# tomstrident/GAN-based-Video-Style-Transfer

Measured on NVIDIA B200. Metric: warped frame-pairs/sec, higher is better.
Workload: dtype f32

## Files before the change

### gan-based-video-style-transfer_b200/_cabi.py

```python
import ctypes
import os
import subprocess

_HERE = os.path.dirname(os.path.abspath(__file__))
CSRC = os.path.join(_HERE, "csrc")
LIB_PATH = os.environ.get("TCL_B200_LIB") or os.path.join(CSRC, "libtcl_b200.so")
HEADER = os.path.join(os.path.dirname(_HERE), "include", "tcl_b200.h")
ABI_VERSION = 6

F32, BF16 = 0, 1
OCC, MOB, VALIDITY = 1, 2, 4
L2, L1 = 0, 1
FIN_MEAN, FIN_RMSE = 0, 1

NVCC_FLAGS = ["-gencode", "arch=compute_100a,code=sm_100a", "-O3", "-lineinfo", "-std=c++17",
              "-Xcompiler", "-fPIC", "-shared"]
SOURCES = ["tcl_kernels.cu", "tcl_host.cu", "tcl_cv2.cu", "tcl_agg.cu", "tcl_chain.cu"]
HEADERS = ["tcl_math.cuh", "tcl_common.cuh"]


class TclArgs(ctypes.Structure):
    _fields_ = [
        ("ff", ctypes.c_void_p), ("bf", ctypes.c_void_p), ("mask_in", ctypes.c_void_p),
        ("prev", ctypes.c_void_p), ("cur", ctypes.c_void_p),
# ... 81 lines not shown
    "tclb200_warp_backward": (_c.c_int, [_vp, _vp, _vp, _vp, _vp, _i, _i, _i, _i, _i, _vp]),
    "tclb200_fbcheck": (_c.c_int, [_vp, _vp, _vp, _i, _i, _i, _i, _vp, _vp]),
    "tclb200_tcl_forward": (_c.c_int, [_c.POINTER(TclArgs), _vp]),
    "tclb200_host_workspace_bytes": (_c.c_size_t, [_i, _i, _i, _i, _i, _i, _i, _i]),
    "tclb200_tcl_forward_host": (_c.c_int, [_c.POINTER(HostArgs), _vp]),
    "tclb200_tcl_backward": (_c.c_int, [_vp, _vp, _vp, _vp, _vp, _vp, _vp, _i, _i, _i, _i, _i, _i, _vp]),
    "tclb200_tcl_backward_scaled": (_c.c_int, [_vp, _vp, _vp, _vp, _vp, _c.c_float, _vp, _vp, _i, _i, _i, _i, _i, _i, _vp]),
    "tclb200_backward_workspace_bytes": (_c.c_size_t, [_i, _i, _i, _i, _i]),
    "tclb200_warp_backward_dt": (_c.c_int, [_vp, _vp, _vp, _vp, _vp, _i, _i, _i, _i, _i, _i, _vp, _c.c_size_t, _vp]),
    "tclb200_tcl_backward_dt": (_c.c_int, [_vp, _vp, _vp, _vp, _vp, _c.c_float, _vp, _vp, _i, _i, _i, _i, _i, _i, _i, _vp,
                                           _c.c_size_t, _vp]),
    "tclb200_hwc_split": (_c.c_int, [_vp, _i, _i, _i, _i, _i, _vp, _vp, _vp, _vp]),
    "tclb200_occlusion_u8_to_mask": (_c.c_int, [_vp, _vp, _c.c_size_t, _vp]),
    "tclb200_upsample_flow": (_c.c_int, [_vp, _vp, _vp, _i, _i, _i, _vp]),
    "tclb200_cv2_remap": (_c.c_int, [_vp, _vp, _vp, _i, _i, _i, _i, _vp]),
    "tclb200_cv2_fb_check": (_c.c_int, [_vp, _vp, _vp, _i, _i, _i, _i, _i, _vp, _vp]),
    "tclb200_reconet_scratch_bytes": (_c.c_size_t, [_i, _i, _i]),
    "tclb200_reconet_loss": (_c.c_int, [_vp, _vp, _vp, _vp, _vp, _vp, _vp, _vp, _vp, _vp, _c.c_size_t, _i, _i, _i, _vp]),
    "tclb200_ruder_input": (_c.c_int, [_vp, _vp, _vp, _vp, _vp, _vp, _i, _i, _i, _vp]),
    "tclb200_pack_sequence_sums": (_c.c_int, [_vp, _vp, _vp, _i, _i, _c.c_double, _vp, _vp]),
    "tclb200_unpack_sequence_means": (_c.c_int, [_vp, _i, _vp, _vp]),
    "tclb200_debug_force_generic": (None, [_i]),
    "tclb200_debug_tile_stats": (_c.c_int, [_vp, _i]),
    "tclb200_debug_launch_count": (_c.c_ulonglong, [_i]),
}

_lib = None


class TclB200Error(RuntimeError):
    pass


def lib():
    global _lib
    if _lib is not None:
        return _lib
    if not os.path.exists(LIB_PATH):
        raise TclB200Error(
            f"{LIB_PATH} is missing: build it with `python -c 'import __graft_entry__ as g; g.build()'` "
            "(nvcc, sm_100a). There is no CPU or PyTorch fallback for this path.")
    handle = ctypes.CDLL(LIB_PATH)
    for name, (res, args) in _PROTOTYPES.items():
        fn = getattr(handle, name)
        fn.restype, fn.argtypes = res, args
    got = handle.tclb200_abi_version()
# ... 19 lines not shown
```

### gan-based-video-style-transfer_b200/csrc/tcl_kernels.cu

```cuda
#include <cuda.h>
#include <cuda_bf16.h>
#include <cuda_runtime.h>
#include <limits.h>
#include <stdint.h>
#include <stdio.h>
#include <string.h>
#include <type_traits>

#include "../../include/tcl_b200.h"
#include "tcl_common.cuh"
#include "tcl_math.cuh"

#ifndef TCL_TH
#define TCL_TH 32
#endif
#ifndef TCL_BH
#define TCL_BH 42
#endif
#ifndef TCL_BH8
#define TCL_BH8 44
#endif
#ifndef TCL_BH16
#define TCL_BH16 TCL_BH
#endif
#ifndef TCL_BW
#define TCL_BW 80
#endif
#ifndef TCL_BW16
#define TCL_BW16 80
#endif
#ifndef TCL_NS
#define TCL_NS 2
#endif
#ifndef TCL_NB
#define TCL_NB (TCL_NS + 2)
#endif
#ifndef TCL_NS_NOFF
#define TCL_NS_NOFF 3
#endif
#ifndef TCL_BH_NOFF
#define TCL_BH_NOFF 40
#endif
#ifndef TCL_SCANNERS
#define TCL_SCANNERS 2
#endif
#ifndef TCL_PACKED
// ... 244 lines not shown
        const float xc = to_f32(s_c[c][ii[q]]);
        if (LOSS == TCLB200_L2) {
          const float md = __fmul_rn(keep[q], __fsub_rn(xc, w[q][c]));
          e = __fmaf_rn(md, md, e);
        } else {
          e = __fadd_rn(e, __fmul_rn(keep[q], fabsf(__fsub_rn(w[q][c], xc))));
        }
      }
      err = ok[q] ? e : err;
    }
  }
  double s = warp_sum((double)err);
  if ((threadIdx.x & 31) == 0) s_red[threadIdx.x >> 5] = s;
  __syncthreads();
  if (threadIdx.x == 0) {
    s = 0.0;
#pragma unroll
    for (int k = 0; k < kDirectThreads / 32; ++k) s += s_red[k];
    __stcg(&p.scratch.partials[(size_t)pair * p.tiles_per_pair + chunk], s);
  }
}

__device__ unsigned long long g_tile_stats[2];
#ifdef TCL_TRACE
constexpr int kTraceTiles = 64;
__device__ unsigned long long g_trace[160][kTraceTiles][4];
__device__ __forceinline__ unsigned long long gtime() { unsigned long long t; asm volatile("mov.u64 %0, %globaltimer;" : "=l"(t)); return t; }
#define TCL_STAMP(k, slot) do { if ((k) < kTraceTiles && blockIdx.x < 160) g_trace[blockIdx.x][(k)][(slot)] = gtime(); } while (0)
#else
#define TCL_STAMP(k, slot) do { } while (0)
#endif
#ifdef TCL_CWARPS
constexpr int kCWarpsPacked = TCL_CWARPS, kCWarpsOther = TCL_CWARPS;
#else
constexpr int kCWarpsPacked = 8, kCWarpsOther = 16;
#endif

template <typename FrameT, int CT, int TW_, int TH_, int BW_, int BH_, int NB_, int NS_, int CW_, bool FF_ = true>
struct WsCfg {
  static constexpr int TW = TW_, TH = TH_, BW = BW_, BH = BH_, NB = NB_, NS = NS_;
  static constexpr int CW = CW_;
  static constexpr int kProducerWarp = CW;
  static constexpr int kScannerWarp = CW + 1;
  static constexpr int kScanners = TCL_SCANNERS;
  static constexpr int kThreads = 32 * (CW + 1 + kScanners);
  static constexpr int kHaloL = 4;
  static constexpr int kBfW = TW + 16, kBfH = TH + 2;
  static constexpr int kXAlign = 16 / (int)sizeof(FrameT);
  static constexpr int kRowBlocks = CW / 4;
  static constexpr int kRows = TH / kRowBlocks;
  static constexpr int kPPL = kRows / 2;
  static constexpr int kC = CT > 0 ? CT : 1;
  static constexpr unsigned kBfLoad = 2u * kBfH * kBfW * 4u;
  static constexpr unsigned kFfLoad = 2u * BH * BW * 4u;
  static constexpr unsigned kPrevLoad = (unsigned)(CT > 0 ? CT : 0) * BH * BW * (unsigned)sizeof(FrameT);
  static constexpr size_t kBfStage = align_up(kBfLoad, 128);
  static constexpr size_t kFfStage = FF_ ? align_up(kFfLoad, 128) : 0;
  static constexpr size_t kSrcStage = kFfStage + align_up(kPrevLoad, 128);
  static constexpr size_t kBfOff = 0;
  static constexpr size_t kSrcOff = kBfOff + NB * kBfStage;
  static constexpr size_t kCtlOff = kSrcOff + NS * kSrcStage;
  static constexpr size_t kCtlBytes = 1024 + (size_t)NS * CW * 32 * 4;
  static constexpr size_t kSmemBytes = kCtlOff + kCtlBytes + 128;
  static_assert(TW == 64 && CW % 4 == 0 && TH % kRowBlocks == 0 && kRows % 2 == 0, "lane mapping: 16-column blocks, row pairs");
  static_assert(kBfW % 32 == 16, "flow-tile pitch must be 16 (mod 32) words: adjacent rows fall into disjoint bank halves");
  static_assert((BW * (int)sizeof(FrameT)) % 16 == 0 && BW % 4 == 0, "TMA: box rows are multiples of 16 bytes");
#if TCL_DIAG != 3
  static_assert(NB >= NS + 1, "the flow tile of a tile is scanned NS tiles ahead of its use");
  static_assert(kSmemBytes <= 232448, "a CTA has at most 227 KB of shared memory");
#endif
};
__host__ __device__ constexpr int pix_dy(int k) { return 2 * k; }
template <typename Cfg>
__device__ __forceinline__ void lane_origin(int warp, int lane, int& lx0, int& ly0) {
  lx0 = 16 * (warp & 3) + (lane & 15);
  ly0 = Cfg::kRows * (warp >> 2) + (lane >> 4);
}

struct TileId { int pair, tile, x0, y0, pf, cf, bfi, ffi; };

template <int NB, int NS, int CW>
struct WsCtl {
  uint64_t bf_full[NB], scanned[NB], src_full[NS], done[NS];
  TileId tinfo[NB];
  int meta[NS][4];
  int box[NB][4];
  float red[NS][CW * 32];
};

// ... 708 lines not shown
                                                                  t.x0 + lx0, t.y0 + ly0 + pix_dy(k), 0.0f, 0.0f, 0.0f, 0.0f);
          keepbits = (keepbits & ~(1u << k)) | ((kp != 0.0f ? 1u : 0u) << k);
        }
      }
  }
  if (CT == 0) {
    float* mo = p.mask_out + (size_t)t.pair * gplane + (size_t)(t.y0 + ly0) * g.W + (t.x0 + lx0);
#pragma unroll
    for (int k = 0; k < P; ++k)
      if (!EDGE || (xin && 2 * k < rows_in)) __stcs(mo + (ptrdiff_t)pix_dy(k) * g.W, ((keepbits >> k) & 1u) ? 1.0f : 0.0f);
    return 0.0f;
  }
  float err = 0.0f;
#pragma unroll
  for (int k = 0; k < P; ++k) {
    if (MASK == MASK_GIVEN) err = __fadd_rn(err, e[k]);
    else err = ((keepbits >> k) & 1u) ? __fadd_rn(err, e[k]) : err;
  }
  return err;
}

template <typename FrameT, int MASK, bool REDUCE, int CT, int LEAN, typename Cfg>
__global__ void __launch_bounds__(Cfg::kThreads, 1) fused_forward_ws_kernel(const FwdParams p, const __grid_constant__ CUtensorMap tm_bf,
                                                                         const __grid_constant__ CUtensorMap tm_ff,
                                                                         const __grid_constant__ CUtensorMap tm_prev,
                                                                         const __grid_constant__ CUtensorMap tm_cur) {
  constexpr int NB = Cfg::NB, NS = Cfg::NS, P = Cfg::kPPL;
  constexpr int kCWarps = Cfg::CW;
  constexpr int kLoss = LEAN == 2 ? TCLB200_L1 : TCLB200_L2;
  constexpr bool kPacked = TCL_PACKED && (((LEAN == 1 || LEAN == 2) && CT == 3 && (MASK == MASK_COMPUTED || (MASK == MASK_GIVEN && TCL_PACKED_GIVEN))) ||
                                          (TCL_PACKED_MASK && LEAN == 1 && CT == 0 && MASK == MASK_COMPUTED && !REDUCE));
  using Ctl = WsCtl<NB, NS, kCWarps>;
  static_assert(sizeof(Ctl) <= Cfg::kCtlBytes, "control block too large");
  extern __shared__ __align__(128) unsigned char smem_raw[];
  unsigned char* smem = smem_raw + ((128u - (smem_u32(smem_raw) & 127u)) & 127u);
  Ctl* ctl = reinterpret_cast<Ctl*>(smem + Cfg::kCtlOff);
  auto bf_stage = [&](int s) { return reinterpret_cast<float*>(smem + Cfg::kBfOff + (size_t)s * Cfg::kBfStage); };
  auto ff_stage = [&](int s) { return reinterpret_cast<float*>(smem + Cfg::kSrcOff + (size_t)s * Cfg::kSrcStage); };
  auto prev_stage = [&](int s) { return reinterpret_cast<FrameT*>(smem + Cfg::kSrcOff + (size_t)s * Cfg::kSrcStage + Cfg::kFfStage); };

  const int total_tiles = p.B * p.tiles_per_pair;
  const bool want_occ = MASK == MASK_COMPUTED && (LEAN ? LEAN != 3 : (p.flags & TCLB200_OCC) != 0);
  const bool want_frames = CT > 0 && (LEAN || p.prev != nullptr);
  const bool want_scan = want_occ || want_frames;
  const int warp = threadIdx.x >> 5, lane = threadIdx.x & 31;
  const Geo& g = p.geo;
  auto real = [&](int k) { return ctl->tinfo[k % NB].pair >= 0; };

  if (REDUCE) asm volatile("griddepcontrol.launch_dependents;" ::: "memory");
// ... 8 lines not shown
    const bool dynamic = p.scratch.tile_ctr != nullptr;
    int tg_next = (int)blockIdx.x;
    bool exhausted = false;
    auto next_tile = [&]() {
      const int tg = tg_next;
      tg_next = dynamic ? (int)gridDim.x + (int)atomicAdd(p.scratch.tile_ctr, 1u) : tg + (int)gridDim.x;
      return tg;
    };
    auto issue_bf = [&](int k) {
      const int s = k % NB;
      const int tg = exhausted ? total_tiles : next_tile();
      if (tg >= total_tiles) {
        exhausted = true;
        ctl->tinfo[s].pair = -1;
        mbar_arrive(&ctl->bf_full[s]);
        return;
      }
      const TileId t = tile_id(p, tg, Cfg::TW, Cfg::TH);
      ctl->tinfo[s] = t;
      mbar_expect_tx(&ctl->bf_full[s], Cfg::kBfLoad);
      tma_load_4d(bf_stage(s), &tm_bf, &ctl->bf_full[s], t.x0 - Cfg::kHaloL, t.y0 - 1, 0, t.bfi);
      if (LEAN && CT > 0 && p.cur != nullptr) tma_prefetch_l2_4d(&tm_cur, t.x0, t.y0, 0, t.cf);
    };
    struct Placement { int ox, oy, mode, ffi, pf; };
    auto place_src = [&](int k) -> Placement {
      const int sb = k % NB;
      const TileId t = ctl->tinfo[sb];
      int ox = 0, oy = 0, mode = 0;
#if TCL_DIAG == 3
      if (true) { ox = (t.x0 - 8) & ~3; oy = t.y0 - 4; mode = 1; } else
#endif
      if (want_scan) {
        mbar_wait_idle(&ctl->scanned[sb], (k / NB) & 1);
        const float xmin = ord2f(ctl->box[sb][0]), ymin = ord2f(ctl->box[sb][1]), xmax = ord2f(ctl->box[sb][2]), ymax = ord2f(ctl->box[sb][3]);
        const float lim = 30000.0f;
        const bool sane = xmin > -lim && xmax < lim && ymin > -lim && ymax < lim && xmin <= xmax && ymin <= ymax;
        if (sane) {
          const float i2x = __fmul_rn(2.0f, g.inv_dx), i2y = __fmul_rn(2.0f, g.inv_dy);
          auto coord = [](float a, float i2, float sz) {
            const float tt = __fadd_rn(__fsub_rn(__fmul_rn(a, i2), 1.0f), 1.0f);
            return __fmul_rn(__fmaf_rn(tt, sz, -1.0f), 0.5f);
          };
          const int bx0 = __float2int_rd(coord(xmin, i2x, g.Wf)), bx1 = __float2int_rd(coord(xmax, i2x, g.Wf));
          const int by0 = __float2int_rd(coord(ymin, i2y, g.Hf)), by1 = __float2int_rd(coord(ymax, i2y, g.Hf));
          ox = bx0 & ~(Cfg::kXAlign - 1);
          oy = by0;
          const bool fitx = bx1 + 1 - ox < Cfg::BW, fity = by1 + 1 - oy < Cfg::BH;
          mode = (fitx && fity) ? 1 : 2;
          if (mode == 2) {
            if (!fitx) ox = ((bx0 + bx1 + 1 - Cfg::BW) / 2) & ~(Cfg::kXAlign - 1);
            if (!fity) oy = (by0 + by1 + 1 - Cfg::BH) / 2;
          }
        }
        if (mode != 1) atomicAdd(&g_tile_stats[mode == 2 ? 1 : 0], 1ull);
      }
      return Placement{ox, oy, mode, t.ffi, t.pf};
    };
    auto issue_src = [&](int k, const Placement& pl) {
      const int ss = k % NS;
      ctl->meta[ss][0] = pl.ox; ctl->meta[ss][1] = pl.oy; ctl->meta[ss][2] = pl.mode;
#if TCL_DIAG == 1
      if (false) {
#else
      if (pl.mode != 0) {
#endif
        TCL_STAMP(k, 0);
        mbar_expect_tx(&ctl->src_full[ss], (want_occ ? Cfg::kFfLoad : 0u) + (want_frames ? Cfg::kPrevLoad : 0u));
        if (want_occ) tma_load_4d(ff_stage(ss), &tm_ff, &ctl->src_full[ss], pl.ox, pl.oy, 0, pl.ffi);
        if (want_frames) tma_load_4d(prev_stage(ss), &tm_prev, &ctl->src_full[ss], pl.ox, pl.oy, 0, pl.pf);
      } else {
        mbar_arrive(&ctl->src_full[ss]);
      }
    };

    if (lane == 0) {
      prefetch_tmap(&tm_bf);
      if (want_occ) prefetch_tmap(&tm_ff);
      if (want_frames) prefetch_tmap(&tm_prev);
      for (int j = 0; j < NB; ++j) issue_bf(j);
      for (int j = 0; j < NS && real(j); ++j) issue_src(j, place_src(j));
    }
    __syncwarp();
    for (int j = 0; real(j); ++j) {
      mbar_wait_idle(&ctl->done[j % NS], (j / NS) & 1);
      const TileId t = ctl->tinfo[j % NB];
      double ts = 0.0;
      if (REDUCE) {
        const float* r = ctl->red[j % NS] + lane;
#pragma unroll
        for (int w = 0; w < kCWarps; ++w) ts += (double)r[32 * w];
      }
      __syncwarp();
      if (lane == 0) {
        if (real(j + NS)) issue_src(j + NS, place_src(j + NS));
        issue_bf(j + NB);
      }
      __syncwarp();
      if (REDUCE) {
        ts = warp_sum(ts);
        if (lane == 0) __stcg(&p.scratch.partials[(size_t)t.pair * p.tiles_per_pair + t.tile], ts);
      }
    }
    if (dynamic && lane == 0) {
      __threadfence();
      if (atomicAdd(p.scratch.tile_ctr + 1, 1u) == gridDim.x - 1) {
        p.scratch.tile_ctr[0] = 0;
        p.scratch.tile_ctr[1] = 0;
      }
    }
    return;
  }

  if (warp >= Cfg::kScannerWarp) {
    if (!want_scan || TCL_DIAG == 3) return;
    for (int k = warp - Cfg::kScannerWarp;; k += Cfg::kScanners) {
      const int sb = k % NB;
      mbar_wait_idle(&ctl->bf_full[sb], (k / NB) & 1);
      if (ctl->tinfo[sb].pair < 0) return;
      scan_flow_tile<Cfg>(bf_stage(sb), ctl->tinfo[sb], g, p.row_end, ctl->box[sb], lane);
      __syncwarp();
      if (lane == 0) mbar_arrive(&ctl->scanned[sb]);
    }
  }

  unsigned near = 0;
// ... 455 lines not shown
  if (!batch_stride) batch_stride = plane_stride * planes;
  const cuuint64_t dims[4] = {(cuuint64_t)W, (cuuint64_t)H, (cuuint64_t)planes, (cuuint64_t)B};
  const cuuint64_t strides[3] = {(cuuint64_t)W * esize, (cuuint64_t)plane_stride * esize, (cuuint64_t)batch_stride * esize};
  const cuuint32_t box[4] = {(cuuint32_t)bw, (cuuint32_t)bh, (cuuint32_t)bp, 1u};
  const cuuint32_t estr[4] = {1u, 1u, 1u, 1u};
  const CUtensorMapDataType dt = esize == 2 ? CU_TENSOR_MAP_DATA_TYPE_BFLOAT16 : CU_TENSOR_MAP_DATA_TYPE_FLOAT32;
  return fn(m, dt, 4, const_cast<void*>(base), dims, strides, box, estr, CU_TENSOR_MAP_INTERLEAVE_NONE,
            CU_TENSOR_MAP_SWIZZLE_NONE, CU_TENSOR_MAP_L2_PROMOTION_L2_256B, CU_TENSOR_MAP_FLOAT_OOB_FILL_NONE) == CUDA_SUCCESS;
}

static int sm_count() {
  static int cache[64] = {};
  int dev = 0, v = 0;
  if (cudaGetDevice(&dev) != cudaSuccess) return 148;
  if (dev >= 0 && dev < 64 && cache[dev] > 0) return cache[dev];
  if (cudaDeviceGetAttribute(&v, cudaDevAttrMultiProcessorCount, dev) != cudaSuccess || v <= 0) return 148;
  if (dev >= 0 && dev < 64) cache[dev] = v;
  return v;
}

static cudaError_t launch_fold(const FwdParams& p, cudaStream_t s);

template <typename FrameT, int MASK, bool REDUCE, int CT, int LEAN, int CW>
static cudaError_t launch_tma_cw(const FwdParams& p, const CUtensorMap& tb, const CUtensorMap& tf, const CUtensorMap& tp, const CUtensorMap& tc,
                                 cudaStream_t s) {
  constexpr bool has_ff = MASK == MASK_COMPUTED;
  constexpr int NS = has_ff ? (CT == 0 && LEAN == 1 ? TCL_NS_MASK : TCL_NS) : TCL_NS_NOFF, NB = has_ff ? (CT == 0 && LEAN == 1 ? TCL_NS_MASK + 2 : TCL_NB) : TCL_NS_NOFF + 2;
  using Cfg = WsCfg<FrameT, CT, kTW, kTH, box_width<FrameT>(), (has_ff ? box_height(CW, (int)sizeof(FrameT)) : TCL_BH_NOFF), NB, NS, CW, has_ff>;
  auto kern = fused_forward_ws_kernel<FrameT, MASK, REDUCE, CT, LEAN, Cfg>;
  static bool configured[64] = {};
  int dev = 0;
  if (cudaGetDevice(&dev) != cudaSuccess || dev < 0 || dev >= 64) dev = 63;
  if (!configured[dev] || dev == 63) {
    cudaError_t e = cudaFuncSetAttribute(kern, cudaFuncAttributeMaxDynamicSharedMemorySize, (int)Cfg::kSmemBytes);
    if (e != cudaSuccess) return e;
    configured[dev] = true;
  }
  const size_t tiles = (size_t)p.B * p.tiles_per_pair;
  const size_t slots = (size_t)sm_count();
  const unsigned grid = (unsigned)(tiles < slots ? tiles : slots);
  kern<<<grid, Cfg::kThreads, Cfg::kSmemBytes, s>>>(p, tb, tf, tp, tc);
  ++g_launches;
  cudaError_t e = cudaGetLastError();
  if (e != cudaSuccess || !REDUCE) return e;
  return launch_fold(p, s);
}

template <typename FrameT, int MASK, bool REDUCE, int CT, int LEAN>
static cudaError_t launch_tma(const FwdParams& p, const CUtensorMap& tb, const CUtensorMap& tf, const CUtensorMap& tp, const CUtensorMap& tc,
                              cudaStream_t s) {
  constexpr bool packed8 = TCL_PACKED && MASK == MASK_COMPUTED && sizeof(FrameT) == 4 &&
                           (((LEAN == 1 || LEAN == 2) && CT == 3) || (TCL_PACKED_MASK && LEAN == 1 && CT == 0 && !REDUCE));
  if constexpr (packed8 && kCWarpsPacked != kCWarpsOther) {
    if (p.cw_packed) return launch_tma_cw<FrameT, MASK, REDUCE, CT, LEAN, kCWarpsPacked>(p, tb, tf, tp, tc, s);
  }
  if (p.cw_packed && kCWarpsPacked != kCWarpsOther) return cudaErrorInvalidConfiguration;
  return launch_tma_cw<FrameT, MASK, REDUCE, CT, LEAN, kCWarpsOther>(p, tb, tf, tp, tc, s);
}

static cudaError_t launch_fold(const FwdParams& p, cudaStream_t s) {
  ++g_launches;
  cudaLaunchConfig_t cfg;
  memset(&cfg, 0, sizeof(cfg));
  const bool small = p.B <= kFoldSmallPairs && (size_t)p.B * p.tiles_per_pair <= (size_t)kFoldSmallPartials;
  cfg.gridDim = dim3(small ? 1u : (unsigned)p.B); cfg.blockDim = dim3(small ? 1024 : kThreads); cfg.stream = s;
  cudaLaunchAttribute attr[1];
  attr[0].id = cudaLaunchAttributeProgrammaticStreamSerialization;
  attr[0].val.programmaticStreamSerializationAllowed = 1;
  cfg.attrs = attr; cfg.numAttrs = 1;
  return small ? cudaLaunchKernelEx(&cfg, fold_partials_small_kernel, p) : cudaLaunchKernelEx(&cfg, fold_partials_kernel, p);
}

template <typename FrameT>
static cudaError_t launch_direct(const FwdParams& p, cudaStream_t s) {
  auto kern = p.loss == TCLB200_L1 ? fused_forward_direct_kernel<FrameT, TCLB200_L1> : fused_forward_direct_kernel<FrameT, TCLB200_L2>;
  kern<<<(unsigned)((size_t)p.B * p.tiles_per_pair), kDirectThreads, 0, s>>>(p);
  ++g_launches;
  cudaError_t e = cudaGetLastError();
  if (e != cudaSuccess) return e;
  return launch_fold(p, s);
}

template <typename FrameT, int MASK, bool REDUCE>
static cudaError_t launch_generic(const FwdParams& p, cudaStream_t s) {
  const unsigned grid = (unsigned)((size_t)p.B * p.tiles_per_pair);
  if (p.C == 3) fused_forward_generic_kernel<FrameT, MASK, REDUCE, 3><<<grid, kThreads, 0, s>>>(p);
  else fused_forward_generic_kernel<FrameT, MASK, REDUCE, 0><<<grid, kThreads, 0, s>>>(p);
  ++g_launches;
  return cudaGetLastError();
}

template <typename FrameT>
static cudaError_t dispatch(const FwdParams& p, int mask_kind, bool reduce, bool tma, const CUtensorMap& tb, const CUtensorMap& tf,
                            const CUtensorMap& tp, const CUtensorMap& tc, cudaStream_t s) {
#ifdef TCL_HOT_ONLY
  if (sizeof(FrameT) == (TCL_HOT_ONLY == 2 ? 2 : 4) && mask_kind == MASK_COMPUTED && reduce && tma && p.C == 3 && p.prev && p.cur && !p.warp_out && !p.mask_out &&
      !p.blend_out && !p.near_threshold && p.loss == TCLB200_L2)
    return launch_tma<typename std::conditional<TCL_HOT_ONLY == 2, __nv_bfloat16, float>::type, MASK_COMPUTED, true, 3, 1>(p, tb, tf, tp, tc, s);
  if (mask_kind == MASK_COMPUTED && !reduce && !p.prev) return launch_generic<float, MASK_COMPUTED, false>(p, s);
  return cudaErrorNotSupported;
#else
#define TCL_CASE(MK, RD)                                                                       \
  if (mask_kind == MK && reduce == RD) {                                                       \
    if (!tma) return launch_generic<FrameT, MK, RD>(p, s);                                     \
    if (p.C == 3 && lean_out && MK != MASK_NONE) return launch_tma<FrameT, (MK == MASK_NONE ? MASK_GIVEN : MK), RD, 3, 4>(p, tb, tf, tp, tc, s); \
    if (p.C == 3 && lean && RD) return p.loss == TCLB200_L1 ? launch_tma<FrameT, MK, true, 3, 2>(p, tb, tf, tp, tc, s)   \
                                                            : launch_tma<FrameT, MK, true, 3, 1>(p, tb, tf, tp, tc, s);  \
    if (MK == MASK_COMPUTED && !RD && lean_mask) return launch_tma<float, MASK_COMPUTED, false, 0, 1>(p, tb, tf, tp, tc, s); \
    if (MK == MASK_COMPUTED && !RD && lean_mob) return launch_tma<float, MASK_COMPUTED, false, 0, 3>(p, tb, tf, tp, tc, s); \
    if (MK == MASK_NONE && !RD && lean_warp) return launch_tma<FrameT, MASK_NONE, false, 3, 1>(p, tb, tf, tp, tc, s); \
    return p.C == 3 ? launch_tma<FrameT, MK, RD, 3, 0>(p, tb, tf, tp, tc, s) : launch_tma<FrameT, MK, RD, 0, 0>(p, tb, tf, tp, tc, s); \
  }
  const bool lean = reduce && p.prev && p.cur && !p.warp_out && !p.mask_out && !p.blend_out && !p.near_threshold &&
                    !(p.flags & TCLB200_VALIDITY) && mask_kind != MASK_NONE &&
                    (mask_kind != MASK_COMPUTED || (p.flags & (TCLB200_OCC | TCLB200_MOB)) == (TCLB200_OCC | TCLB200_MOB));
  const bool lean_out = p.prev && p.cur && (p.warp_out || p.blend_out || (p.mask_out && mask_kind == MASK_COMPUTED)) &&
                        !(p.mask_out && mask_kind == MASK_GIVEN) && !p.near_threshold && !(p.flags & TCLB200_VALIDITY) &&
                        p.loss == TCLB200_L2 && mask_kind != MASK_NONE &&
                        (mask_kind != MASK_COMPUTED || (p.flags & (TCLB200_OCC | TCLB200_MOB)) == (TCLB200_OCC | TCLB200_MOB));
  const bool lean_mask = !reduce && !p.prev && p.mask_out && !p.near_threshold && mask_kind == MASK_COMPUTED &&
                         (p.flags & (TCLB200_OCC | TCLB200_MOB)) == (TCLB200_OCC | TCLB200_MOB);
  const bool lean_mob = !reduce && !p.prev && p.mask_out && !p.near_threshold && mask_kind == MASK_COMPUTED &&
                        (p.flags & (TCLB200_OCC | TCLB200_MOB)) == TCLB200_MOB;
  const bool lean_warp = !reduce && p.prev && p.C == 3 && !p.cur && p.warp_out && !p.mask_out && !p.blend_out && mask_kind == MASK_NONE;
  TCL_CASE(MASK_COMPUTED, true)
  TCL_CASE(MASK_COMPUTED, false)
  TCL_CASE(MASK_GIVEN, true)
  TCL_CASE(MASK_GIVEN, false)
  TCL_CASE(MASK_NONE, true)
  TCL_CASE(MASK_NONE, false)
#undef TCL_CASE
  return cudaErrorInvalidValue;
#endif
}

extern "C" int tclb200_debug_tile_stats(unsigned long long* out2, int reset) {
  unsigned long long zero[2] = {0, 0};
  if (out2) CUDA_TRY(cudaMemcpyFromSymbol(out2, tcl::g_tile_stats, sizeof(zero)));
  if (reset) CUDA_TRY(cudaMemcpyToSymbol(tcl::g_tile_stats, zero, sizeof(zero)));
  return TCLB200_OK;
}

extern "C" unsigned long long tclb200_debug_launch_count(int reset) {
  const unsigned long long n = g_launches;
  if (reset) g_launches = 0;
  return n;
}

#ifdef TCL_TRACE
extern "C" int tclb200_debug_trace(unsigned long long* out, size_t bytes) {
  if (bytes > sizeof(tcl::g_trace)) bytes = sizeof(tcl::g_trace);
  CUDA_TRY(cudaMemcpyFromSymbol(out, tcl::g_trace, bytes));
  return TCLB200_OK;
}
#endif

static int g_force_generic = 0;
extern "C" void tclb200_debug_force_generic(int on) { g_force_generic = on; }
#ifndef TCL_DIRECT_MAX_PX
#define TCL_DIRECT_MAX_PX (2u << 20)
#endif

// ... 23 lines not shown
    return fail(TCLB200_ERR_INVALID, "ff given but neither TCLB200_OCC nor TCLB200_MOB requested");
  if (!a->prev && !a->mask_out) return fail(TCLB200_ERR_INVALID, "nothing to compute: no frames and no mask_out");

  const int esz = a->dtype == TCLB200_BF16 ? 2 : 4;
  const size_t hw = (size_t)a->H * a->W;
  const size_t bf_plane = a->bf_plane_stride ? a->bf_plane_stride : hw, bf_batch = a->bf_batch_stride ? a->bf_batch_stride : 2 * bf_plane;
  const size_t ff_plane = a->ff_plane_stride ? a->ff_plane_stride : hw, ff_batch = a->ff_batch_stride ? a->ff_batch_stride : 2 * ff_plane;
  if (bf_plane < hw || ff_plane < hw || (a->B > 1 && (bf_batch < hw || ff_batch < hw)))
    return fail(TCLB200_ERR_INVALID, "flow plane / pair strides must be at least H*W");
  const bool strides16 = bf_plane % 4 == 0 && bf_batch % 4 == 0 && ff_plane % 4 == 0 && ff_batch % 4 == 0;
  bool tma = g_force_generic != 1 && (a->W % 4 == 0) && ((a->W * esz) % 16 == 0) && aligned16(a->bf) && aligned16(a->ff) &&
             aligned16(a->prev) && aligned16(a->cur) && (!a->prev || a->C == 3) && a->B <= 65535 * 16 && strides16 &&
             a->H <= 16384 && a->W <= 16384;
  const bool cw_hot = reduce && a->prev && a->cur && a->C == 3 && !a->warp_out && !a->mask_out && !a->blend_out;
  const bool cw_mask = TCL_PACKED_MASK && !reduce && !a->prev && a->mask_out;
  const bool cw_packed = TCL_PACKED && kCWarpsPacked != kCWarpsOther && tma && a->dtype == TCLB200_F32 && mask_kind == MASK_COMPUTED &&
                         (cw_hot || cw_mask) && !a->near_threshold &&
                         !(a->flags & TCLB200_VALIDITY) && (a->flags & (TCLB200_OCC | TCLB200_MOB)) == (TCLB200_OCC | TCLB200_MOB) &&
                         (size_t)a->H * a->W >= (size_t)384 * 384;
  const size_t launch_px = (size_t)a->B * (size_t)((band ? a->row_end - a->row_begin : a->H)) * a->W;
  const bool direct = tma && g_force_generic != 2 && mask_kind == MASK_GIVEN && reduce && a->C == 3 && !a->warp_out && !a->mask_out &&
                      !a->blend_out && !a->near_threshold && !(a->flags & (TCLB200_VALIDITY | TCLB200_THROUGHPUT)) && aligned16(a->mask_in) &&
                      (launch_px <= TCL_DIRECT_MAX_PX || g_force_generic == 3);
  CUtensorMap tb, tf, tp, tc;
  memset(&tb, 0, sizeof(tb)); memset(&tf, 0, sizeof(tf)); memset(&tp, 0, sizeof(tp)); memset(&tc, 0, sizeof(tc));
  if (tma && !direct) {
    const int bw = a->dtype == TCLB200_BF16 ? box_width<__nv_bfloat16>() : box_width<float>();
    const int kBH = mask_kind == MASK_COMPUTED ? box_height(cw_packed ? kCWarpsPacked : kCWarpsOther, esz) : TCL_BH_NOFF;
    tma = make_map(&tb, a->bf, 4, a->W, a->H, 2, a->bf_index ? a->n_bf_fields : a->B, kTW + 16, kTH + 2, 2, bf_plane, bf_batch);
    if (tma && mask_kind == MASK_COMPUTED && (a->flags & TCLB200_OCC))
      tma = make_map(&tf, a->ff, 4, a->W, a->H, 2, a->ff_index ? a->n_ff_fields : a->B, bw, kBH, 2, ff_plane, ff_batch);
    if (tma && a->prev) tma = make_map(&tp, a->prev, esz, a->W, a->H, 3, a->prev_index ? a->n_prev_frames : a->B, bw, kBH, 3);
    if (tma && a->prev && a->cur) tma = make_map(&tc, a->cur, esz, a->W, a->H, 3, a->cur_index ? a->n_cur_frames : a->B, kTW, kTH, 3);
  }

  FwdParams p;
  memset(&p, 0, sizeof(p));
  p.ff = a->ff; p.bf = a->bf; p.mask_in = a->mask_in; p.prev = a->prev; p.cur = a->cur;
  p.ff_plane = ff_plane; p.ff_batch = ff_batch; p.bf_plane = bf_plane; p.bf_batch = bf_batch;
  p.prev_index = a->prev ? a->prev_index : nullptr; p.cur_index = a->cur ? a->cur_index : nullptr;
  p.bf_index = a->bf_index; p.ff_index = a->ff ? a->ff_index : nullptr;
  p.pair_group = a->pair_group > 1 ? a->pair_group : 1;
  p.cw_packed = cw_packed ? 1 : 0;
  p.warp_out = a->warp_out; p.mask_out = a->mask_out; p.blend_out = a->blend_out;
  p.pair_sums = a->pair_sums; p.total_sums = a->total_sums; p.pair_vals = a->pair_vals; p.total_val = a->total_val;
  p.near_threshold = a->near_threshold;
  p.geo = make_geo(a->H, a->W);
  p.B = a->B; p.C = a->prev ? a->C : 0;
  p.row_begin = band ? a->row_begin : 0;
  p.row_end = band ? a->row_end : a->H;
  p.tiles_x = tma ? cdiv(a->W, kTW) : cdiv(a->W, 32);
  p.tiles_per_pair = p.tiles_x * (tma ? cdiv(p.row_end - p.row_begin, kTH) : cdiv(p.row_end - p.row_begin, kWarps));
  if (direct) { p.tiles_x = 0; p.tiles_per_pair = (int)(((size_t)(p.row_end - p.row_begin) * a->W + kDirectChunk - 1) / kDirectChunk); }
  p.flags = a->flags; p.loss = a->loss; p.finalize = a->finalize;
  p.inv_count = a->prev ? 1.0 / ((double)a->C * a->H * a->W) : 0.0;
  if ((size_t)p.B * p.tiles_per_pair >= 0x7fffffffu) return fail(TCLB200_ERR_UNSUPPORTED, "too many tiles for one launch");
  if (reduce) {
    if (!a->scratch || a->scratch_bytes < tclb200_scratch_bytes(a->B, a->H, a->W))
      return fail(TCLB200_ERR_INVALID, "scratch missing or smaller than tclb200_scratch_bytes(B,H,W)");
    char* base = reinterpret_cast<char*>(a->scratch);
    const size_t tpp_max = (size_t)cdiv(a->W, 32) * cdiv(a->H, kWarps);
    p.scratch.partials = reinterpret_cast<double*>(base);
    p.scratch.pair_ticket = reinterpret_cast<unsigned*>(base + align_up((size_t)a->B * tpp_max * sizeof(double), 256));
    p.scratch.batch_ticket = p.scratch.pair_ticket + a->B;
    const size_t tiles = (size_t)p.B * p.tiles_per_pair;
    p.scratch.tile_ctr = (tma && !direct && tiles > 16 * (size_t)sm_count()) ? p.scratch.batch_ticket + 1 : nullptr;
  }
  if (direct) {
    const cudaError_t e = a->dtype == TCLB200_BF16 ? launch_direct<__nv_bfloat16>(p, s) : launch_direct<float>(p, s);
    if (e != cudaSuccess) return fail(TCLB200_ERR_CUDA, "fused forward (direct) launch: %s", cudaGetErrorString(e));
    return TCLB200_OK;
  }
  const cudaError_t e = a->dtype == TCLB200_BF16 ? dispatch<__nv_bfloat16>(p, mask_kind, reduce, tma, tb, tf, tp, tc, s)
                                                 : dispatch<float>(p, mask_kind, reduce, tma, tb, tf, tp, tc, s);
  if (e != cudaSuccess) return fail(TCLB200_ERR_CUDA, "fused forward launch: %s", cudaGetErrorString(e));
  return TCLB200_OK;
}

extern "C" int tclb200_tcl_forward(const tclb200_tcl_args* args, tclb200_stream_t stream) {
  return run_fused(args, reinterpret_cast<cudaStream_t>(stream));
}

extern "C" int tclb200_warp(const void* x, const float* f, void* out, int B, int C, int H, int W, int dtype, int flags,
                            tclb200_stream_t stream) {
  if (!x || !f || !out) return fail(TCLB200_ERR_INVALID, "x, f and out are required");
  tclb200_tcl_args a;
  memset(&a, 0, sizeof(a));
  a.bf = f; a.prev = x; a.warp_out = out;
  a.B = B; a.C = C; a.H = H; a.W = W; a.dtype = dtype; a.flags = flags & TCLB200_VALIDITY;
  return run_fused(&a, reinterpret_cast<cudaStream_t>(stream));
}

extern "C" int tclb200_fbcheck(const float* ff, const float* bf, float* mask_out, int B, int H, int W, int flags,
                               unsigned long long* near_threshold, tclb200_stream_t stream) {
  if (!bf || !mask_out) return fail(TCLB200_ERR_INVALID, "bf and mask_out are required");
  if ((flags & TCLB200_OCC) && !ff) return fail(TCLB200_ERR_INVALID, "ff is required for the occlusion test");
  if (!(flags & (TCLB200_OCC | TCLB200_MOB))) return fail(TCLB200_ERR_INVALID, "flags must request TCLB200_OCC and/or TCLB200_MOB");
// ... 200 lines not shown
```

### include/tcl_b200.h

```cpp
#ifndef TCL_B200_H_
#define TCL_B200_H_

#include <stddef.h>
#include <stdint.h>

#ifdef __cplusplus
extern "C" {
#endif

#define TCLB200_ABI_VERSION 6

#define TCLB200_OK 0
#define TCLB200_ERR_INVALID 1
#define TCLB200_ERR_CUDA 2
#define TCLB200_ERR_UNSUPPORTED 3

#define TCLB200_F32 0
#define TCLB200_BF16 1

#define TCLB200_OCC 1
#define TCLB200_MOB 2
#define TCLB200_VALIDITY 4
#define TCLB200_THROUGHPUT 8

// ... 97 lines not shown
int tclb200_occlusion_u8_to_mask(const uint8_t* src, float* dst, size_t n, tclb200_stream_t stream);

int tclb200_upsample_flow(const float* flow, const float* mask, float* out, int N, int H, int W, tclb200_stream_t stream);

int tclb200_cv2_remap(const float* src, const float* flow, float* out, int N, int H, int W, int C, tclb200_stream_t stream);
int tclb200_cv2_fb_check(const float* ff, const float* bf, float* mask, int N, int H, int W, int flags, int prewarped,
                         unsigned long long* near_threshold, tclb200_stream_t stream);

size_t tclb200_reconet_scratch_bytes(int B, int H, int W);
int tclb200_reconet_loss(const float* flow, const float* mask, const float* styled1, const float* styled2, const float* img1,
                         const float* img2, float* lum_out, float* loss_out, double* sum_out, void* scratch, size_t scratch_bytes,
                         int B, int H, int W, tclb200_stream_t stream);
int tclb200_ruder_input(const float* img, const float* mask, const float* styled_prev, const float* flow, float* cat_out,
                        float* warp_out, int B, int H, int W, tclb200_stream_t stream);

int tclb200_pack_sequence_sums(const float* pair_vals, const double* sum_sq, const long long* seq_of_pair, int n_pairs, int n_seq,
                               double elems_per_pair, double* packed, tclb200_stream_t stream);
int tclb200_unpack_sequence_means(const double* packed, int n_seq, double* out, tclb200_stream_t stream);

void tclb200_debug_force_generic(int on);

int tclb200_debug_tile_stats(unsigned long long* out2, int reset);

unsigned long long tclb200_debug_launch_count(int reset);

#ifdef __cplusplus
}
#endif
#endif
```

Baseline: 251,000.

## Stage source tiles with variable-height TMA boxes sized to the flow footprint

Builds three tensor maps per source (forward flow and previous frame) with box heights stepping down by 4 rows. Per tile, the producer picks the shortest box that covers the warped footprint rows and issues per-channel loads for that box only. The point is to cut TMA bytes moved into shared memory when the displacement range is small. In exchange it issues more TMA instructions (one per channel), passes a larger parameter struct, and adds global atomic counters for staged rows. BH16 is also set to 44.

Result: no change. 250,500, median of 6 (-0.2%).

```diff
diff --git a/gan-based-video-style-transfer_b200/_cabi.py b/gan-based-video-style-transfer_b200/_cabi.py
--- a/gan-based-video-style-transfer_b200/_cabi.py
+++ b/gan-based-video-style-transfer_b200/_cabi.py
@@ -127,6 +127,7 @@
     "tclb200_unpack_sequence_means": (_c.c_int, [_vp, _i, _vp, _vp]),
     "tclb200_debug_force_generic": (None, [_i]),
     "tclb200_debug_tile_stats": (_c.c_int, [_vp, _i]),
+    "tclb200_debug_box_rows": (_c.c_int, [_vp, _i]),
     "tclb200_debug_launch_count": (_c.c_ulonglong, [_i]),
 }
 
diff --git a/gan-based-video-style-transfer_b200/csrc/tcl_kernels.cu b/gan-based-video-style-transfer_b200/csrc/tcl_kernels.cu
--- a/gan-based-video-style-transfer_b200/csrc/tcl_kernels.cu
+++ b/gan-based-video-style-transfer_b200/csrc/tcl_kernels.cu
@@ -21,7 +21,7 @@
 #define TCL_BH8 44
 #endif
 #ifndef TCL_BH16
-#define TCL_BH16 TCL_BH
+#define TCL_BH16 44
 #endif
 #ifndef TCL_BW
 #define TCL_BW 80
@@ -312,6 +312,7 @@
 }
 
 __device__ unsigned long long g_tile_stats[2];
+__device__ unsigned long long g_box_rows[2];
 #ifdef TCL_TRACE
 constexpr int kTraceTiles = 64;
 __device__ unsigned long long g_trace[160][kTraceTiles][4];
@@ -325,6 +326,12 @@
 #else
 constexpr int kCWarpsPacked = 8, kCWarpsOther = 16;
 #endif
+
+constexpr int kBoxHeights = 3, kBoxStep = 4;
+__host__ __device__ constexpr int box_rows(int bh, int c) { return bh - (kBoxHeights - 1 - c) * kBoxStep; }
+struct SrcMaps {
+  CUtensorMap ff[kBoxHeights], prev[kBoxHeights];
+};
 
 template <typename FrameT, int CT, int TW_, int TH_, int BW_, int BH_, int NB_, int NS_, int CW_, bool FF_ = true>
 struct WsCfg {
@@ -342,8 +349,10 @@
   static constexpr int kPPL = kRows / 2;
   static constexpr int kC = CT > 0 ? CT : 1;
   static constexpr unsigned kBfLoad = 2u * kBfH * kBfW * 4u;
-  static constexpr unsigned kFfLoad = 2u * BH * BW * 4u;
-  static constexpr unsigned kPrevLoad = (unsigned)(CT > 0 ? CT : 0) * BH * BW * (unsigned)sizeof(FrameT);
+  __host__ __device__ static constexpr int rows(int c) { return box_rows(BH, c); }
+  static constexpr unsigned kFfRow = 2u * BW * 4u, kPrevRow = (unsigned)(CT > 0 ? CT : 0) * BW * (unsigned)sizeof(FrameT);
+  static constexpr unsigned kFfLoad = BH * kFfRow;
+  static constexpr unsigned kPrevLoad = BH * kPrevRow;
   static constexpr size_t kBfStage = align_up(kBfLoad, 128);
   static constexpr size_t kFfStage = FF_ ? align_up(kFfLoad, 128) : 0;
   static constexpr size_t kSrcStage = kFfStage + align_up(kPrevLoad, 128);
@@ -355,6 +364,8 @@
   static_assert(TW == 64 && CW % 4 == 0 && TH % kRowBlocks == 0 && kRows % 2 == 0, "lane mapping: 16-column blocks, row pairs");
   static_assert(kBfW % 32 == 16, "flow-tile pitch must be 16 (mod 32) words: adjacent rows fall into disjoint bank halves");
   static_assert((BW * (int)sizeof(FrameT)) % 16 == 0 && BW % 4 == 0, "TMA: box rows are multiples of 16 bytes");
+  static_assert(rows(0) >= 2, "discarded pixels read the taps of the box origin: rows 0 and 1 are always staged");
+  static_assert((BH * BW * (int)sizeof(FrameT)) % 128 == 0, "TMA: every plane of a stage starts on a 128-byte boundary");
 #if TCL_DIAG != 3
   static_assert(NB >= NS + 1, "the flow tile of a tile is scanned NS tiles ahead of its use");
   static_assert(kSmemBytes <= 232448, "a CTA has at most 227 KB of shared memory");
@@ -1109,9 +1120,8 @@
 
 template <typename FrameT, int MASK, bool REDUCE, int CT, int LEAN, typename Cfg>
 __global__ void __launch_bounds__(Cfg::kThreads, 1) fused_forward_ws_kernel(const FwdParams p, const __grid_constant__ CUtensorMap tm_bf,
-                                                                         const __grid_constant__ CUtensorMap tm_ff,
-                                                                         const __grid_constant__ CUtensorMap tm_prev,
-                                                                         const __grid_constant__ CUtensorMap tm_cur) {
+                                                                         const __grid_constant__ CUtensorMap tm_cur,
+                                                                         const __grid_constant__ SrcMaps tm_src) {
   constexpr int NB = Cfg::NB, NS = Cfg::NS, P = Cfg::kPPL;
   constexpr int kCWarps = Cfg::CW;
   constexpr int kLoss = LEAN == 2 ? TCLB200_L1 : TCLB200_L2;
@@ -1166,11 +1176,13 @@
       tma_load_4d(bf_stage(s), &tm_bf, &ctl->bf_full[s], t.x0 - Cfg::kHaloL, t.y0 - 1, 0, t.bfi);
       if (LEAN && CT > 0 && p.cur != nullptr) tma_prefetch_l2_4d(&tm_cur, t.x0, t.y0, 0, t.cf);
     };
-    struct Placement { int ox, oy, mode, ffi, pf; };
+    struct Placement { int ox, oy, mode, hc, ffi, pf; };
+    unsigned long long staged_tiles = 0, staged_rows = 0;
     auto place_src = [&](int k) -> Placement {
       const int sb = k % NB;
       const TileId t = ctl->tinfo[sb];
       int ox = 0, oy = 0, mode = 0;
+      int hc = kBoxHeights - 1;
 #if TCL_DIAG == 3
       if (true) { ox = (t.x0 - 8) & ~3; oy = t.y0 - 4; mode = 1; } else
 #endif
@@ -1191,6 +1203,8 @@
           oy = by0;
           const bool fitx = bx1 + 1 - ox < Cfg::BW, fity = by1 + 1 - oy < Cfg::BH;
           mode = (fitx && fity) ? 1 : 2;
+          if (mode == 1)
+            while (hc > 0 && Cfg::rows(hc - 1) >= by1 + 2 - oy) --hc;
           if (mode == 2) {
             if (!fitx) ox = ((bx0 + bx1 + 1 - Cfg::BW) / 2) & ~(Cfg::kXAlign - 1);
             if (!fity) oy = (by0 + by1 + 1 - Cfg::BH) / 2;
@@ -1198,7 +1212,7 @@
         }
         if (mode != 1) atomicAdd(&g_tile_stats[mode == 2 ? 1 : 0], 1ull);
       }
-      return Placement{ox, oy, mode, t.ffi, t.pf};
+      return Placement{ox, oy, mode, hc, t.ffi, t.pf};
     };
     auto issue_src = [&](int k, const Placement& pl) {
       const int ss = k % NS;
@@ -1209,9 +1223,24 @@
       if (pl.mode != 0) {
 #endif
         TCL_STAMP(k, 0);
-        mbar_expect_tx(&ctl->src_full[ss], (want_occ ? Cfg::kFfLoad : 0u) + (want_frames ? Cfg::kPrevLoad : 0u));
-        if (want_occ) tma_load_4d(ff_stage(ss), &tm_ff, &ctl->src_full[ss], pl.ox, pl.oy, 0, pl.ffi);
-        if (want_frames) tma_load_4d(prev_stage(ss), &tm_prev, &ctl->src_full[ss], pl.ox, pl.oy, 0, pl.pf);
+        const int h = Cfg::rows(pl.hc);
+        constexpr int PL = Cfg::BH * Cfg::BW;
+#if TCL_DIAG == 4
+        {
+          const float qnan = __int_as_float(0x7fffffff);
+          for (int c = 0; want_occ && c < 2; ++c)
+            for (int i = h * Cfg::BW; i < PL; ++i) ff_stage(ss)[c * PL + i] = qnan;
+          for (int c = 0; want_frames && c < Cfg::kC; ++c)
+            for (int i = h * Cfg::BW; i < PL; ++i) prev_stage(ss)[c * PL + i] = (FrameT)qnan;
+          asm volatile("fence.proxy.async.shared::cta;" ::: "memory");
+        }
+#endif
+        staged_tiles += 1; staged_rows += (unsigned)h;
+        mbar_expect_tx(&ctl->src_full[ss], (unsigned)h * ((want_occ ? Cfg::kFfRow : 0u) + (want_frames ? Cfg::kPrevRow : 0u)));
+        if (want_occ)
+          for (int c = 0; c < 2; ++c) tma_load_4d(ff_stage(ss) + c * PL, &tm_src.ff[pl.hc], &ctl->src_full[ss], pl.ox, pl.oy, c, pl.ffi);
+        if (want_frames)
+          for (int c = 0; c < Cfg::kC; ++c) tma_load_4d(prev_stage(ss) + c * PL, &tm_src.prev[pl.hc], &ctl->src_full[ss], pl.ox, pl.oy, c, pl.pf);
       } else {
         mbar_arrive(&ctl->src_full[ss]);
       }
@@ -1219,8 +1248,10 @@
 
     if (lane == 0) {
       prefetch_tmap(&tm_bf);
-      if (want_occ) prefetch_tmap(&tm_ff);
-      if (want_frames) prefetch_tmap(&tm_prev);
+      for (int c = 0; c < kBoxHeights; ++c) {
+        if (want_occ) prefetch_tmap(&tm_src.ff[c]);
+        if (want_frames) prefetch_tmap(&tm_src.prev[c]);
+      }
       for (int j = 0; j < NB; ++j) issue_bf(j);
       for (int j = 0; j < NS && real(j); ++j) issue_src(j, place_src(j));
     }
@@ -1245,6 +1276,7 @@
         if (lane == 0) __stcg(&p.scratch.partials[(size_t)t.pair * p.tiles_per_pair + t.tile], ts);
       }
     }
+    if (lane == 0 && staged_tiles != 0) { atomicAdd(&g_box_rows[0], staged_tiles); atomicAdd(&g_box_rows[1], staged_rows); }
     if (dynamic && lane == 0) {
       __threadfence();
       if (atomicAdd(p.scratch.tile_ctr + 1, 1u) == gridDim.x - 1) {
@@ -1746,8 +1778,7 @@
 static cudaError_t launch_fold(const FwdParams& p, cudaStream_t s);
 
 template <typename FrameT, int MASK, bool REDUCE, int CT, int LEAN, int CW>
-static cudaError_t launch_tma_cw(const FwdParams& p, const CUtensorMap& tb, const CUtensorMap& tf, const CUtensorMap& tp, const CUtensorMap& tc,
-                                 cudaStream_t s) {
+static cudaError_t launch_tma_cw(const FwdParams& p, const CUtensorMap& tb, const CUtensorMap& tc, const SrcMaps& ts, cudaStream_t s) {
   constexpr bool has_ff = MASK == MASK_COMPUTED;
   constexpr int NS = has_ff ? (CT == 0 && LEAN == 1 ? TCL_NS_MASK : TCL_NS) : TCL_NS_NOFF, NB = has_ff ? (CT == 0 && LEAN == 1 ? TCL_NS_MASK + 2 : TCL_NB) : TCL_NS_NOFF + 2;
   using Cfg = WsCfg<FrameT, CT, kTW, kTH, box_width<FrameT>(), (has_ff ? box_height(CW, (int)sizeof(FrameT)) : TCL_BH_NOFF), NB, NS, CW, has_ff>;
@@ -1763,7 +1794,7 @@
   const size_t tiles = (size_t)p.B * p.tiles_per_pair;
   const size_t slots = (size_t)sm_count();
   const unsigned grid = (unsigned)(tiles < slots ? tiles : slots);
-  kern<<<grid, Cfg::kThreads, Cfg::kSmemBytes, s>>>(p, tb, tf, tp, tc);
+  kern<<<grid, Cfg::kThreads, Cfg::kSmemBytes, s>>>(p, tb, tc, ts);
   ++g_launches;
   cudaError_t e = cudaGetLastError();
   if (e != cudaSuccess || !REDUCE) return e;
@@ -1771,15 +1802,14 @@
 }
 
 template <typename FrameT, int MASK, bool REDUCE, int CT, int LEAN>
-static cudaError_t launch_tma(const FwdParams& p, const CUtensorMap& tb, const CUtensorMap& tf, const CUtensorMap& tp, const CUtensorMap& tc,
-                              cudaStream_t s) {
+static cudaError_t launch_tma(const FwdParams& p, const CUtensorMap& tb, const CUtensorMap& tc, const SrcMaps& ts, cudaStream_t s) {
   constexpr bool packed8 = TCL_PACKED && MASK == MASK_COMPUTED && sizeof(FrameT) == 4 &&
                            (((LEAN == 1 || LEAN == 2) && CT == 3) || (TCL_PACKED_MASK && LEAN == 1 && CT == 0 && !REDUCE));
   if constexpr (packed8 && kCWarpsPacked != kCWarpsOther) {
-    if (p.cw_packed) return launch_tma_cw<FrameT, MASK, REDUCE, CT, LEAN, kCWarpsPacked>(p, tb, tf, tp, tc, s);
+    if (p.cw_packed) return launch_tma_cw<FrameT, MASK, REDUCE, CT, LEAN, kCWarpsPacked>(p, tb, tc, ts, s);
   }
   if (p.cw_packed && kCWarpsPacked != kCWarpsOther) return cudaErrorInvalidConfiguration;
-  return launch_tma_cw<FrameT, MASK, REDUCE, CT, LEAN, kCWarpsOther>(p, tb, tf, tp, tc, s);
+  return launch_tma_cw<FrameT, MASK, REDUCE, CT, LEAN, kCWarpsOther>(p, tb, tc, ts, s);
 }
 
 static cudaError_t launch_fold(const FwdParams& p, cudaStream_t s) {
@@ -1815,25 +1845,25 @@
 }
 
 template <typename FrameT>
-static cudaError_t dispatch(const FwdParams& p, int mask_kind, bool reduce, bool tma, const CUtensorMap& tb, const CUtensorMap& tf,
-                            const CUtensorMap& tp, const CUtensorMap& tc, cudaStream_t s) {
+static cudaError_t dispatch(const FwdParams& p, int mask_kind, bool reduce, bool tma, const CUtensorMap& tb, const CUtensorMap& tc,
+                            const SrcMaps& ts, cudaStream_t s) {
 #ifdef TCL_HOT_ONLY
   if (sizeof(FrameT) == (TCL_HOT_ONLY == 2 ? 2 : 4) && mask_kind == MASK_COMPUTED && reduce && tma && p.C == 3 && p.prev && p.cur && !p.warp_out && !p.mask_out &&
       !p.blend_out && !p.near_threshold && p.loss == TCLB200_L2)
-    return launch_tma<typename std::conditional<TCL_HOT_ONLY == 2, __nv_bfloat16, float>::type, MASK_COMPUTED, true, 3, 1>(p, tb, tf, tp, tc, s);
+    return launch_tma<typename std::conditional<TCL_HOT_ONLY == 2, __nv_bfloat16, float>::type, MASK_COMPUTED, true, 3, 1>(p, tb, tc, ts, s);
   if (mask_kind == MASK_COMPUTED && !reduce && !p.prev) return launch_generic<float, MASK_COMPUTED, false>(p, s);
   return cudaErrorNotSupported;
 #else
 #define TCL_CASE(MK, RD)                                                                       \
   if (mask_kind == MK && reduce == RD) {                                                       \
     if (!tma) return launch_generic<FrameT, MK, RD>(p, s);                                     \
-    if (p.C == 3 && lean_out && MK != MASK_NONE) return launch_tma<FrameT, (MK == MASK_NONE ? MASK_GIVEN : MK), RD, 3, 4>(p, tb, tf, tp, tc, s); \
-    if (p.C == 3 && lean && RD) return p.loss == TCLB200_L1 ? launch_tma<FrameT, MK, true, 3, 2>(p, tb, tf, tp, tc, s)   \
-                                                            : launch_tma<FrameT, MK, true, 3, 1>(p, tb, tf, tp, tc, s);  \
-    if (MK == MASK_COMPUTED && !RD && lean_mask) return launch_tma<float, MASK_COMPUTED, false, 0, 1>(p, tb, tf, tp, tc, s); \
-    if (MK == MASK_COMPUTED && !RD && lean_mob) return launch_tma<float, MASK_COMPUTED, false, 0, 3>(p, tb, tf, tp, tc, s); \
-    if (MK == MASK_NONE && !RD && lean_warp) return launch_tma<FrameT, MASK_NONE, false, 3, 1>(p, tb, tf, tp, tc, s); \
-    return p.C == 3 ? launch_tma<FrameT, MK, RD, 3, 0>(p, tb, tf, tp, tc, s) : launch_tma<FrameT, MK, RD, 0, 0>(p, tb, tf, tp, tc, s); \
+    if (p.C == 3 && lean_out && MK != MASK_NONE) return launch_tma<FrameT, (MK == MASK_NONE ? MASK_GIVEN : MK), RD, 3, 4>(p, tb, tc, ts, s); \
+    if (p.C == 3 && lean && RD) return p.loss == TCLB200_L1 ? launch_tma<FrameT, MK, true, 3, 2>(p, tb, tc, ts, s)   \
+                                                            : launch_tma<FrameT, MK, true, 3, 1>(p, tb, tc, ts, s);  \
+    if (MK == MASK_COMPUTED && !RD && lean_mask) return launch_tma<float, MASK_COMPUTED, false, 0, 1>(p, tb, tc, ts, s); \
+    if (MK == MASK_COMPUTED && !RD && lean_mob) return launch_tma<float, MASK_COMPUTED, false, 0, 3>(p, tb, tc, ts, s); \
+    if (MK == MASK_NONE && !RD && lean_warp) return launch_tma<FrameT, MASK_NONE, false, 3, 1>(p, tb, tc, ts, s); \
+    return p.C == 3 ? launch_tma<FrameT, MK, RD, 3, 0>(p, tb, tc, ts, s) : launch_tma<FrameT, MK, RD, 0, 0>(p, tb, tc, ts, s); \
   }
   const bool lean = reduce && p.prev && p.cur && !p.warp_out && !p.mask_out && !p.blend_out && !p.near_threshold &&
                     !(p.flags & TCLB200_VALIDITY) && mask_kind != MASK_NONE &&
@@ -1862,6 +1892,13 @@
   unsigned long long zero[2] = {0, 0};
   if (out2) CUDA_TRY(cudaMemcpyFromSymbol(out2, tcl::g_tile_stats, sizeof(zero)));
   if (reset) CUDA_TRY(cudaMemcpyToSymbol(tcl::g_tile_stats, zero, sizeof(zero)));
+  return TCLB200_OK;
+}
+
+extern "C" int tclb200_debug_box_rows(unsigned long long* out2, int reset) {
+  unsigned long long zero[2] = {0, 0};
+  if (out2) CUDA_TRY(cudaMemcpyFromSymbol(out2, tcl::g_box_rows, sizeof(zero)));
+  if (reset) CUDA_TRY(cudaMemcpyToSymbol(tcl::g_box_rows, zero, sizeof(zero)));
   return TCLB200_OK;
 }
 
@@ -1931,15 +1968,18 @@
   const bool direct = tma && g_force_generic != 2 && mask_kind == MASK_GIVEN && reduce && a->C == 3 && !a->warp_out && !a->mask_out &&
                       !a->blend_out && !a->near_threshold && !(a->flags & (TCLB200_VALIDITY | TCLB200_THROUGHPUT)) && aligned16(a->mask_in) &&
                       (launch_px <= TCL_DIRECT_MAX_PX || g_force_generic == 3);
-  CUtensorMap tb, tf, tp, tc;
-  memset(&tb, 0, sizeof(tb)); memset(&tf, 0, sizeof(tf)); memset(&tp, 0, sizeof(tp)); memset(&tc, 0, sizeof(tc));
+  CUtensorMap tb, tc;
+  SrcMaps ts;
+  memset(&tb, 0, sizeof(tb)); memset(&tc, 0, sizeof(tc)); memset(&ts, 0, sizeof(ts));
   if (tma && !direct) {
     const int bw = a->dtype == TCLB200_BF16 ? box_width<__nv_bfloat16>() : box_width<float>();
     const int kBH = mask_kind == MASK_COMPUTED ? box_height(cw_packed ? kCWarpsPacked : kCWarpsOther, esz) : TCL_BH_NOFF;
     tma = make_map(&tb, a->bf, 4, a->W, a->H, 2, a->bf_index ? a->n_bf_fields : a->B, kTW + 16, kTH + 2, 2, bf_plane, bf_batch);
-    if (tma && mask_kind == MASK_COMPUTED && (a->flags & TCLB200_OCC))
-      tma = make_map(&tf, a->ff, 4, a->W, a->H, 2, a->ff_index ? a->n_ff_fields : a->B, bw, kBH, 2, ff_plane, ff_batch);
-    if (tma && a->prev) tma = make_map(&tp, a->prev, esz, a->W, a->H, 3, a->prev_index ? a->n_prev_frames : a->B, bw, kBH, 3);
+    for (int c = 0; c < kBoxHeights; ++c) {
+      if (tma && mask_kind == MASK_COMPUTED && (a->flags & TCLB200_OCC))
+        tma = make_map(&ts.ff[c], a->ff, 4, a->W, a->H, 2, a->ff_index ? a->n_ff_fields : a->B, bw, box_rows(kBH, c), 1, ff_plane, ff_batch);
+      if (tma && a->prev) tma = make_map(&ts.prev[c], a->prev, esz, a->W, a->H, 3, a->prev_index ? a->n_prev_frames : a->B, bw, box_rows(kBH, c), 1);
+    }
     if (tma && a->prev && a->cur) tma = make_map(&tc, a->cur, esz, a->W, a->H, 3, a->cur_index ? a->n_cur_frames : a->B, kTW, kTH, 3);
   }
 
@@ -1980,8 +2020,8 @@
     if (e != cudaSuccess) return fail(TCLB200_ERR_CUDA, "fused forward (direct) launch: %s", cudaGetErrorString(e));
     return TCLB200_OK;
   }
-  const cudaError_t e = a->dtype == TCLB200_BF16 ? dispatch<__nv_bfloat16>(p, mask_kind, reduce, tma, tb, tf, tp, tc, s)
-                                                 : dispatch<float>(p, mask_kind, reduce, tma, tb, tf, tp, tc, s);
+  const cudaError_t e = a->dtype == TCLB200_BF16 ? dispatch<__nv_bfloat16>(p, mask_kind, reduce, tma, tb, tc, ts, s)
+                                                 : dispatch<float>(p, mask_kind, reduce, tma, tb, tc, ts, s);
   if (e != cudaSuccess) return fail(TCLB200_ERR_CUDA, "fused forward launch: %s", cudaGetErrorString(e));
   return TCLB200_OK;
 }
diff --git a/include/tcl_b200.h b/include/tcl_b200.h
--- a/include/tcl_b200.h
+++ b/include/tcl_b200.h
@@ -143,6 +143,8 @@
 
 int tclb200_debug_tile_stats(unsigned long long* out2, int reset);
 
+int tclb200_debug_box_rows(unsigned long long* out2, int reset);
+
 unsigned long long tclb200_debug_launch_count(int reset);
 
 #ifdef __cplusplus
```
